# UltronAI/Depth-VO-Feat

Hardware: AMD Instinct MI355X
Metric: KITTI 256x832 stereo-seq samples/sec fwd+bwd (higher is better)
Workload: dtype f32

## Files before the change

__graft_entry__.py:

```python
import os
import subprocess
import sys

ROOT = os.path.dirname(os.path.abspath(__file__))
PKG = os.path.join(ROOT, "depth-vo-feat_amd")


def _paths():
    for p in (PKG, ROOT):
        if p not in sys.path:
            sys.path.insert(0, p)


def build():
    subprocess.run(["make", "-C", os.path.join(PKG, "csrc"), "-j4"], check=True)
    subprocess.run(["make", "-C", os.path.join(PKG, "csrc"), "TUNING=1", "-j4"], check=True)
    assert os.path.exists(os.path.join(PKG, "dvf", "libdvf_hip_tuning.so"))
    _paths()
    from dvf import lib as L
    lib = L.lib()
    assert lib.dvf_version() >= 100
    import DispNetS, PoseExpNet, PoseExpNet_sfm, inverse_warp, loss_functions, loss_functions_sfm
    import dvf.engine, dvf.steps


def smoke():
    _paths()
    import torch
    from oracle import nets as onets
    from oracle import steps as osteps
    import DispNetS
    import PoseExpNet
    from dvf.engine import FlatAdam
    from dvf.steps import unsupervise_losses
    from dvf.synthetic import synthetic_batch
    assert torch.cuda.is_available(), "smoke() needs the GPU: the product path has no CPU fallback"
    dev = torch.device("cuda:0")
    b, h, w = 1, 64, 128
    dsd = onets.fill_params(onets.dispnet_layers(), seed=1)
    psd = onets.fill_params(onets.posenet_layers(6, 6, 2, True), seed=2)
    disp, pose = DispNetS.DispNetS(), PoseExpNet.PoseExpNet(output_exp=True)
    disp.load_state_dict({k: v.clone() for k, v in dsd.items()})
    pose.load_state_dict({k: v.clone() for k, v in psd.items()})
    disp.to(dev).train()
    pose.to(dev).train()
    opt = FlatAdam(list(pose.parameters()) + list(disp.parameters()), lr=1e-3, weight_decay=1e-8)
    loss, terms = unsupervise_losses(disp, pose, synthetic_batch(b, h, w, seed=1234, device=dev))
    opt.zero_grad()
    loss.backward()
    opt.step()
    torch.cuda.synchronize()
    ref, _, _ = osteps.step_unsupervise(dsd, psd, osteps.synthetic_batch(b, h, w, seed=1234))
    for k in ("img", "smooth", "total"):
        err = abs(float(terms[k]) - float(ref[k])) / abs(float(ref[k]))
        assert err < 1e-4, (k, float(terms[k]), float(ref[k]))
    for name, net, sd in (("disp", disp, dsd), ("pose", pose, psd)):
        for k, v in net.state_dict().items():
            n0 = float(sd[k].double().norm())
            assert abs(float(v.double().norm().cpu()) - n0) <= 1e-4 * max(n0, 1e-12), (name, k)
    print("smoke ok: loss %.6f (oracle %.6f)" % (float(terms["total"]), float(ref["total"])))


if __name__ == "__main__":
    build()
    if "--smoke" in sys.argv:
        smoke()
```

depth-vo-feat_amd/csrc/conv_pipe.h:

```cpp
#pragma once
#include "dvf_common.h"
#include "conv_epilogue.h"

namespace dvfp {

#ifdef DVF_TUNING
#define DVF_STAMP(a, var) do { if ((a).stamps) asm volatile("s_memtime %0\n\ts_waitcnt lgkmcnt(0)" : "=s"(var) :: "memory"); } while (0)
#define DVF_STAMP_RT(a, var) do { if ((a).stamps) asm volatile("s_memrealtime %0\n\ts_waitcnt lgkmcnt(0)" : "=s"(var) :: "memory"); } while (0)
#define DVF_STAMPS_ON 1
#else
#define DVF_STAMP(a, var) do { } while (0)
#define DVF_STAMP_RT(a, var) do { } while (0)
#define DVF_STAMPS_ON 0
#endif

typedef __attribute__((address_space(3))) void lds_void_t;

__device__ __forceinline__ __amdgpu_buffer_rsrc_t tensor_rsrc(const void *p) {
    const uint64_t v = reinterpret_cast<uint64_t>(p);
    const unsigned lo = __builtin_amdgcn_readfirstlane((unsigned)v), hi = __builtin_amdgcn_readfirstlane((unsigned)(v >> 32));
    return __builtin_amdgcn_make_buffer_rsrc(reinterpret_cast<void *>(((uint64_t)hi << 32) | lo), 0, 0x7FFFFFF0, 0x00020000);
}
constexpr unsigned OOB = 0x80000000u;
__device__ __forceinline__ float bload(__amdgpu_buffer_rsrc_t r, unsigned voff, unsigned soff) {
    return __builtin_bit_cast(float, __builtin_amdgcn_raw_buffer_load_b32(r, voff, soff, 0));
}

struct PClass { int py, px, by, bx, TA, TB, OHc, OWc, SL, NTG; unsigned wp_off; };

struct PipeArgs {
    const float *in[DVF_MAX_SEGS];
    int segC[DVF_MAX_SEGS];
    int nseg;
    const float *wp;
    const float *bias;
    float *out;
    int M, N, IH, IW, OH, OW;
    int OS, IS, ncls;
    PClass cls[4];
    int act;
    float alpha, beta;
    int KS, NCH, out_mode, NG;
    int64_t ws_slice;
    int lsw, lsh, TGX, TGY, BW, BH, BN, tilesX, tilesY;
    int x4;
    int blk;
    int SLmax, PSRmax, NST;
    int dbg;
    unsigned long long *stamps;
    const float *mask;
};

__host__ __device__ inline int pipe_row_stride(int RSu, int SW, int SH, int IS) {
    if (SH == 1 || SW >= 32 || (SW % IS) != 0) return RSu;
    const int mod = 32 / IS, want = (SW / IS) % mod;
    const int padded = RSu + ((want - RSu % mod) + mod) % mod;
    return (padded * 8 <= RSu * 9) ? padded : RSu;
}

struct PipeGeo { int PH, PW, PWH, RS, PSR, NPI, XA; };
__host__ __device__ inline PipeGeo pipe_geo(int BH, int BW, int BN, int IS, int TA, int TB, int SW, int SH, int x4 = 0, int bx = 0) {
    PipeGeo g;
    g.PH = (BH - 1) * IS + TA;
    g.PW = (BW - 1) * IS + TB;
    g.PWH = (g.PW + 1) >> 1;
    g.XA = 0;
    if (x4) {
        g.XA = ((bx % 4) + 4) % 4;
        int rs = (g.XA + g.PW + 3) & ~3;
        if (SH > 1 && SW < 32 && (SW & 3) == 0) {
            int padded = rs;
            while (((padded * IS) & 31) != ((SW * IS) & 31) && padded < rs + 32) padded += 4;
            if (((padded * IS) & 31) == ((SW * IS) & 31) && padded * 8 <= rs * 9) rs = padded;
        }
        g.RS = rs;
        g.PSR = (BN * g.PH * g.RS + 255) & ~255;
        g.NPI = g.PSR >> 8;
        return g;
    }
    g.RS = pipe_row_stride(IS == 2 ? 2 * g.PWH : g.PW, SW, SH, IS);
    g.PSR = (BN * g.PH * g.RS + 63) & ~63;
    g.NPI = g.PSR >> 6;
    return g;
}

template <int V> struct fvec;
template <> struct fvec<1> { typedef float type; };
template <> struct fvec<2> { typedef float type __attribute__((ext_vector_type(2))); };
template <> struct fvec<4> { typedef float type __attribute__((ext_vector_type(4))); };

constexpr int PIPE_THREADS = 384;
constexpr int PIPE_THREADS_4P = 512;
constexpr int PIPE_MAXNPI = 32;

template <int MT, int NT, int WM, int CKH, int TBU, int BLK = 0, int NPMAX = PIPE_MAXNPI>
__global__ __launch_bounds__(PIPE_THREADS_4P) __attribute__((amdgpu_waves_per_eu(NPMAX < PIPE_MAXNPI ? 4 : 0)))
void conv_pipe_kernel(const PipeArgs a) {
    constexpr int CK = 2 * CKH, VW = CKH >= 4 ? 4 : CKH, CPG = CKH / VW, MTW = MT * WM;
    constexpr int UNITF = TBU * MTW * 64 * VW;
    static_assert(NPMAX >= 6 && NPMAX <= PIPE_MAXNPI, "by_np dispatches exact piece counts up to 6");
    typedef typename fvec<VW>::type avec;
    extern __shared__ __attribute__((aligned(16))) float smem[];
    const int stage_floats = a.SLmax + CK * a.PSRmax;
    const int tid = threadIdx.x, lane = tid & 63, nl = lane & 31, kh = lane >> 5;
    const int wave = __builtin_amdgcn_readfirstlane(tid >> 6);
    const int zper = gridDim.z / a.ncls;
    const int zc = blockIdx.z / zper, zr = blockIdx.z - zc * zper;
    const int ng = zr / a.KS, ks = zr - ng * a.KS;
    const PClass c = a.cls[zc];
    const int tX = blockIdx.x % a.tilesX, tY = blockIdx.x / a.tilesX;
    const int oy0 = tY * a.BH, ox0 = tX * a.BW, n0 = ng * a.BN;
    if (oy0 >= c.OHc || ox0 >= c.OWc) return;
    const int mb = blockIdx.y;
    const int SW = 1 << a.lsw, SH = 1 << a.lsh;
    const PipeGeo geo = pipe_geo(a.BH, a.BW, a.BN, a.IS, c.TA, TBU, SW, SH, a.x4, c.bx);
    const int RS = geo.RS, PSR = geo.PSR, PWH = geo.PWH;
    const int g_begin = (int)(((int64_t)a.NCH * ks) / a.KS), g_end = (int)(((int64_t)a.NCH * (ks + 1)) / a.KS);
    unsigned long long t_entry = 0, r_entry = 0;
    const int lin_block = (blockIdx.z * gridDim.y + blockIdx.y) * gridDim.x + blockIdx.x;
    DVF_STAMP(a, t_entry);
    DVF_STAMP_RT(a, r_entry);

    if (wave >= 4) {
        auto U = [](int v) __attribute__((always_inline)) { return __builtin_amdgcn_readfirstlane(v); };
        __builtin_amdgcn_s_setprio(3);
        const int nprod = U((int)(blockDim.x >> 6) - 4), pidx = wave - 4;
        const int par = U(nprod == 2 ? pidx : (pidx >> 1));
        const int half = U(nprod == 2 ? 0 : (pidx & 1)), nhalf = U(nprod == 2 ? 1 : 2);
        const int NWP = U(c.SL >> 8);
        const int iy0 = U(oy0 * a.IS + c.by), ix0 = U(ox0 * a.IS + c.bx);
        const int sfl = U(stage_floats), PSRu = U(PSR), NPIu = U(geo.NPI), SLu = U(c.SL), SLmaxu = U(a.SLmax);
        const unsigned wbase = (unsigned)U((int)(c.wp_off + (unsigned)(mb * a.NCH) * (unsigned)c.SL));
        const __amdgpu_buffer_rsrc_t rs_w = tensor_rsrc(a.wp);
        auto issue_w = [&](int g, int st) __attribute__((always_inline)) {
            if (DVF_DBG(a, 2)) return;
            float *wl = smem + st * sfl;
            unsigned so = ((wbase + (unsigned)g * (unsigned)SLu) << 2) + ((unsigned)half << 10);
            float *dst = wl + (half << 8);
            for (int p = half; p < NWP; p += nhalf) {
                __builtin_amdgcn_raw_ptr_buffer_load_lds(rs_w, (lds_void_t *)dst, 16, (unsigned)lane << 4, so, 0, 0);
                so += (unsigned)nhalf << 10;
                dst += nhalf << 8;
            }
        };
        const int D = U(a.NST - 1), nchunks = U(g_end - g_begin), g0 = U(g_begin);
        auto stage_of = [&](int x) __attribute__((always_inline)) { return D == 1 ? (x & 1) : x % 3; };
        if DVF_DBG(a, 8) return;
        for (int x = 0; x < D; ++x)
            if (x < nchunks && (x & 1) == par) issue_w(g0 + x, stage_of(x));

        unsigned pvf[NPMAX];
        unsigned pbn4[(NPMAX + 3) / 4];
#pragma unroll
        for (int q = 0; q < (NPMAX + 3) / 4; ++q) pbn4[q] = 0u;
        {
            const int per_img = geo.PH * RS;
            const float inv_img = 1.0f / (float)per_img, inv_rs = 1.0f / (float)RS;
#pragma unroll
            for (int kk = 0; kk < NPMAX; ++kk) {
                pvf[kk] = OOB;
                if (kk < NPIu) {
                    const int p = a.x4 ? (((kk << 6) + lane) << 2) : ((kk << 6) + lane);
                    int bn = (int)((float)p * inv_img);
                    bn += (p - bn * per_img >= per_img) - (p - bn * per_img < 0);
                    const int rem = p - bn * per_img;
                    int row = (int)((float)rem * inv_rs);
                    row += (rem - row * RS >= RS) - (rem - row * RS < 0);
                    const int col = rem - row * RS;
                    int cs = col - geo.XA;
                    bool ok = (bn < a.BN) && (n0 + bn < a.N);
                    if (a.IS == 2 && !a.x4) {
                        cs = col < PWH ? 2 * col : 2 * (col - PWH) + 1;
                        ok = ok && (col < 2 * PWH);
                    }
                    if (!a.x4) ok = ok && (cs < geo.PW);
                    const int iy = iy0 + row, ix = ix0 + cs;
                    ok = ok && (iy >= 0) && (iy < a.IH) && (ix >= 0) && (ix < a.IW);
                    pvf[kk] = ok ? (unsigned)((iy * a.IW + ix) << 2) : OOB;
                    pbn4[kk >> 2] |= (ok ? (unsigned)bn : 0u) << ((kk & 3) * 8);
                }
            }
        }
        const __amdgpu_buffer_rsrc_t rs_zero = __builtin_amdgcn_make_buffer_rsrc(
            const_cast<float *>(a.wp), 0, 0, 0x00020000);
        const unsigned plane = (unsigned)U((a.IH * a.IW) << 2);
        int iseg = -1, iseg_first = 0, iseg_end = 0, segc = 0;
        __amdgpu_buffer_rsrc_t rs_in = rs_zero;
        unsigned img_cur = 0u;
        auto enter_segment = [&](int g) __attribute__((always_inline)) {
            while (g >= iseg_end) {
                ++iseg;
                iseg_first = iseg_end;
                iseg_end += (a.segC[iseg] + CK - 1) / CK;
            }
            iseg = U(iseg); iseg_first = U(iseg_first); iseg_end = U(iseg_end);
            segc = U(a.segC[iseg]);
            rs_in = tensor_rsrc(a.in[iseg]);
            const unsigned img = (unsigned)segc * plane;
            if (a.BN > 1) {
                const unsigned delta = img - img_cur;
#pragma unroll
                for (int kk = 0; kk < NPMAX; ++kk)
                    if (kk < NPIu) pvf[kk] = (pvf[kk] >> 31) ? OOB : pvf[kk] + ((pbn4[kk >> 2] >> ((kk & 3) * 8)) & 255u) * delta;
            }
            img_cur = img;
        };
        auto issue_p = [&](int g, int st, auto lanec, auto npc, auto exactc) __attribute__((always_inline)) {
            constexpr int LB = decltype(lanec)::value, NP = decltype(npc)::value;
            constexpr bool EXACT = decltype(exactc)::value;
            constexpr int PSH = LB == 16 ? 8 : 6;
            if (g >= iseg_end) enter_segment(g);
            const int c0 = U((g - iseg_first) * CK);
            const int nch = U(min(CK, segc - c0));
            float *dst = smem + st * sfl + SLmaxu + half * PSRu;
            unsigned soff = (unsigned)U((int)((unsigned)(n0 * segc + c0 + half) * plane));
            auto dma = [&](__amdgpu_buffer_rsrc_t r, float *d, unsigned vo, unsigned so) __attribute__((always_inline)) {
                if constexpr (LB == 16) __builtin_amdgcn_raw_ptr_buffer_load_lds(r, (lds_void_t *)d, 16, vo, so, 0, 0);
                else __builtin_amdgcn_raw_ptr_buffer_load_lds(r, (lds_void_t *)d, 4, vo, so, 0, 0);
            };
            int ci = half;
            if (DVF_DBG(a, 32)) {
                for (; ci < nch; ci += nhalf) {
#pragma unroll
                    for (int kk = 0; kk < NP; ++kk)
                        if (EXACT || kk < NPIu) dma(rs_in, dst + (kk << PSH), (unsigned)lane * LB, (unsigned)(kk << (PSH + 2)));
                    dst += nhalf * PSRu;
                }
            }
            for (; ci < nch; ci += nhalf) {
#pragma unroll
                for (int kk = 0; kk < NP; ++kk)
                    if (EXACT || kk < NPIu) dma(rs_in, dst + (kk << PSH), pvf[kk], soff);
                dst += nhalf * PSRu;
                soff += (unsigned)nhalf * plane;
            }
            for (; ci < CK; ci += nhalf) {
#pragma unroll
                for (int kk = 0; kk < NP; ++kk)
                    if (EXACT || kk < NPIu) dma(rs_zero, dst + (kk << PSH), pvf[kk], 0u);
                dst += nhalf * PSRu;
            }
        };
        using std::integral_constant;
        unsigned long long p0 = 0, p1 = 0, p2 = 0, p3 = 0, w_vm = 0, w_bar = 0, w_iss = 0;
        auto chunk_loop = [&](auto lanec, auto npc, auto exactc) __attribute__((always_inline)) {
            if (!DVF_DBG(a, 1))
                for (int x = 0; x < D; ++x)
                    if (x < nchunks && (x & 1) == par) issue_p(g0 + x, stage_of(x), lanec, npc, exactc);
            for (int x = 0; x < nchunks; ++x) {
                DVF_STAMP(a, p0);
                if ((x & 1) == par) asm volatile("s_waitcnt vmcnt(0)" ::: "memory");
                DVF_STAMP(a, p1);
                __builtin_amdgcn_s_barrier();
                DVF_STAMP(a, p2);
                const int nx = x + D;
                if (nx < nchunks && (nx & 1) == par) {
                    issue_w(g0 + nx, stage_of(nx));
                    if (!DVF_DBG(a, 1)) issue_p(g0 + nx, stage_of(nx), lanec, npc, exactc);
                }
                DVF_STAMP(a, p3);
                w_vm += p1 - p0; w_bar += p2 - p1; w_iss += p3 - p2;
            }
        };
        auto by_np = [&](auto lanec) __attribute__((always_inline)) {
            switch (NPIu) {
                case 1: chunk_loop(lanec, integral_constant<int, 1>{}, std::true_type{}); break;
                case 2: chunk_loop(lanec, integral_constant<int, 2>{}, std::true_type{}); break;
                case 3: chunk_loop(lanec, integral_constant<int, 3>{}, std::true_type{}); break;
                case 4: chunk_loop(lanec, integral_constant<int, 4>{}, std::true_type{}); break;
                case 5: chunk_loop(lanec, integral_constant<int, 5>{}, std::true_type{}); break;
                case 6: chunk_loop(lanec, integral_constant<int, 6>{}, std::true_type{}); break;
                default:
                    if constexpr (NPMAX > 12) {
                        if (NPIu <= 12) chunk_loop(lanec, integral_constant<int, 12>{}, std::false_type{});
                        else chunk_loop(lanec, integral_constant<int, NPMAX>{}, std::false_type{});
                    } else {
                        chunk_loop(lanec, integral_constant<int, NPMAX>{}, std::false_type{});
                    }
            }
        };
        if (a.x4) by_np(integral_constant<int, 16>{});
        else by_np(integral_constant<int, 4>{});
        if (DVF_STAMPS_ON && a.stamps && pidx == 0 && lane == 0) {
            a.stamps[8 * lin_block + 5] = w_vm; a.stamps[8 * lin_block + 6] = w_bar; a.stamps[8 * lin_block + 7] = w_iss;
        }
        return;
    }

    const int wm = wave % WM, wn = wave / WM;
    float *bias_lds = smem + a.NST * stage_floats;
    if (tid < 32 * MTW) {
        const int mm = mb * (32 * MTW) + tid;
        bias_lds[tid] = (a.bias && a.out_mode == OUT_FUSED && mm < a.M) ? a.bias[mm] : 0.f;
    }
    const int NU = c.NTG * CPG;
    int opy[NT], opx[NT], opn[NT];
    constexpr bool LR = NPMAX < PIPE_MAXNPI;
    int bj[NT][LR ? 1 : VW];
    const int pxl = nl & (SW - 1), pyl = (nl >> a.lsw) & (SH - 1), pnl = nl >> (a.lsw + a.lsh);
    auto tile_pos = [&](int i, int pxv, int pyv, int pnv) __attribute__((always_inline)) {
        const int q = wn * NT + i, tx = q % a.TGX, tyn = q / a.TGX, ty = tyn % a.TGY, tn = tyn / a.TGY;
        const int SN = 32 >> (a.lsw + a.lsh);
        opy[i] = ty * SH + pyv;
        opx[i] = tx * SW + pxv;
        opn[i] = tn * SN + pnv;
    };
#pragma unroll
    for (int i = 0; i < NT; ++i) {
        tile_pos(i, pxl, pyl, pnl);
        const int bbase = kh * PSR + (opn[i] * geo.PH + opy[i] * a.IS) * RS + (a.x4 ? geo.XA + opx[i] * a.IS : opx[i]);
#pragma unroll
        for (int j = 0; j < (LR ? 1 : VW); ++j) bj[i][j] = bbase + j * 2 * PSR;
    }
    f32x16 acc[MT][NT];
    f32x16 asum[BLK ? MT : 1][BLK ? NT : 1];
#pragma unroll
    for (int m = 0; m < MT; ++m)
#pragma unroll
        for (int i = 0; i < NT; ++i)
#pragma unroll
            for (int r = 0; r < 16; ++r) {
                acc[m][i][r] = 0.f;
                if constexpr (BLK) asum[m][i][r] = 0.f;
            }

    auto consume = [&](int st, auto isc, auto tbec) {
        constexpr int IS = decltype(isc)::value, TBE = decltype(tbec)::value;
        const float *wl = smem + st * stage_floats;
        const float *patch = wl + a.SLmax;
        const float *ap = wl + (wm * MT) * 64 * VW + lane * VW;
        avec af[2][MT];
        float bf[2][TBE][NT][VW];
        int lta = 0, lcpg = 0, lk = 0;
        auto load_bj = [&](auto bufc, auto jc) {
            constexpr int buf = decltype(bufc)::value, j = decltype(jc)::value;
            const float *prow0 = patch + (lta * RS + (lcpg * (2 * VW) + (LR ? 2 * j : 0)) * PSR);
#pragma unroll
            for (int i = 0; i < NT; ++i) {
                const float *prow = prow0 + bj[i][LR ? 0 : j];
                if constexpr (IS == 1) {
#pragma unroll
                    for (int u = 0; u < TBE; ++u) bf[buf][u][i][j] = prow[u];
                } else {
                    const float *prow2 = prow + PWH;
#pragma unroll
                    for (int u = 0; u < TBE; ++u) bf[buf][u][i][j] = (u & 1) ? prow2[u >> 1] : prow[u >> 1];
                }
            }
        };
        auto load_b = [&](auto bufc) {
            load_bj(bufc, std::integral_constant<int, 0>{});
            if constexpr (VW > 1) load_bj(bufc, std::integral_constant<int, 1>{});
            if constexpr (VW > 2) load_bj(bufc, std::integral_constant<int, 2>{});
            if constexpr (VW > 3) load_bj(bufc, std::integral_constant<int, 3>{});
        };
        auto load_a = [&](auto tpc, int unit, auto uc) {
            constexpr int tp = decltype(tpc)::value, u = decltype(uc)::value;
            const float *aptr = ap + unit * UNITF;
#pragma unroll
            for (int m = 0; m < MT; ++m) af[tp][m] = *reinterpret_cast<const avec *>(aptr + (u * MTW + m) * 64 * VW);
        };
        auto advance = [&]() {
            ++lk;
            const bool wrap = (lcpg + 1 == CPG);
            lcpg = wrap ? 0 : lcpg + 1;
            lta += wrap ? 1 : 0;
        };
        auto mma_j = [&](auto bufc, auto tpc, auto uc, auto jc) {
            constexpr int buf = decltype(bufc)::value, tp = decltype(tpc)::value, u = decltype(uc)::value, j = decltype(jc)::value;
#pragma unroll
            for (int m = 0; m < MT; ++m) {
                float av;
                if constexpr (VW == 1) av = af[tp][m]; else av = af[tp][m][j];
#pragma unroll
                for (int i = 0; i < NT; ++i)
                    acc[m][i] = __builtin_amdgcn_mfma_f32_32x32x2f32(av, bf[buf][u][i][j], acc[m][i], 0, 0, 0);
            }
        };
        using B0 = std::integral_constant<int, 0>;
        using B1 = std::integral_constant<int, 1>;
        auto step = [&](auto bufc, auto nbufc, auto pbc, auto uc) {
            constexpr int u = decltype(uc)::value, tp = (decltype(pbc)::value + u) & 1;
            using TP = std::integral_constant<int, tp>;
            mma_j(bufc, TP{}, uc, std::integral_constant<int, 0>{});
            __builtin_amdgcn_sched_barrier(0);
            if constexpr (u + 1 < TBE) load_a(std::integral_constant<int, tp ^ 1>{}, lk - 1, std::integral_constant<int, u + 1>{});
            else load_a(std::integral_constant<int, tp ^ 1>{}, lk, std::integral_constant<int, 0>{});
            if constexpr (u == 0) load_bj(nbufc, std::integral_constant<int, 0>{});
            __builtin_amdgcn_sched_barrier(0);
            if constexpr (VW > 1) {
                mma_j(bufc, TP{}, uc, std::integral_constant<int, 1>{});
                __builtin_amdgcn_sched_barrier(0);
                if constexpr (u == 0) { load_bj(nbufc, std::integral_constant<int, 1>{}); __builtin_amdgcn_sched_barrier(0); }
            }
            if constexpr (VW > 2) {
                mma_j(bufc, TP{}, uc, std::integral_constant<int, 2>{});
                __builtin_amdgcn_sched_barrier(0);
                if constexpr (u == 0) { load_bj(nbufc, std::integral_constant<int, 2>{}); __builtin_amdgcn_sched_barrier(0); }
            }
            if constexpr (VW > 3) {
                mma_j(bufc, TP{}, uc, std::integral_constant<int, 3>{});
                __builtin_amdgcn_sched_barrier(0);
                if constexpr (u == 0) { load_bj(nbufc, std::integral_constant<int, 3>{}); __builtin_amdgcn_sched_barrier(0); }
            }
        };
        auto unit = [&](auto bufc, auto nbufc, auto pbc) {
            step(bufc, nbufc, pbc, std::integral_constant<int, 0>{});
            if constexpr (TBE > 1) step(bufc, nbufc, pbc, std::integral_constant<int, 1>{});
            if constexpr (TBE > 2) step(bufc, nbufc, pbc, std::integral_constant<int, 2>{});
            if constexpr (TBE > 3) step(bufc, nbufc, pbc, std::integral_constant<int, 3>{});
            if constexpr (TBE > 4) step(bufc, nbufc, pbc, std::integral_constant<int, 4>{});
            if constexpr (TBE > 5) step(bufc, nbufc, pbc, std::integral_constant<int, 5>{});
            if constexpr (TBE > 6) step(bufc, nbufc, pbc, std::integral_constant<int, 6>{});
            advance();
        };
        load_b(B0{});
        load_a(B0{}, 0, std::integral_constant<int, 0>{});
        advance();
        __builtin_amdgcn_sched_barrier(0);
        for (int k = 0; k < NU; k += 2) {
            unit(B0{}, B1{}, std::integral_constant<int, 0>{});
            if (k + 1 < NU) unit(B1{}, B0{}, std::integral_constant<int, TBE & 1>{});
        }
    };

    unsigned long long t_loop0 = 0, t_loop1 = 0, tb0 = 0, tb1 = 0, w_bar = 0;
    DVF_STAMP(a, t_loop0);
    if (!DVF_DBG(a, 8)) {
        using IS1 = std::integral_constant<int, 1>;
        using IS2 = std::integral_constant<int, 2>;
        using TBfull = std::integral_constant<int, TBU>;
        using TBless = std::integral_constant<int, (TBU > 1 ? TBU - 1 : 1)>;
        if constexpr (LR) {
            static_assert(!BLK, "the low-register form has no second accumulator set");
            auto chunks = [&](auto isc, auto tbec) __attribute__((always_inline)) {
                int st = 0;
                for (int g = g_begin; g < g_end; ++g) {
                    DVF_STAMP(a, tb0);
                    __syncthreads();
                    DVF_STAMP(a, tb1);
                    w_bar += tb1 - tb0;
                    if (!DVF_DBG(a, 4)) consume(st, isc, tbec);
                    st = (st + 1 == a.NST) ? 0 : st + 1;
                }
            };
            if (a.IS == 2 && !a.x4) chunks(IS2{}, TBfull{});
            else if (TBU > 1 && c.TB == TBU - 1 && !DVF_DBG(a, 64)) chunks(IS1{}, TBless{});
            else chunks(IS1{}, TBfull{});
        } else {
            int st = 0, since = 0;
            for (int g = g_begin; g < g_end; ++g) {
                DVF_STAMP(a, tb0);
                __syncthreads();
                DVF_STAMP(a, tb1);
                w_bar += tb1 - tb0;
                if (!DVF_DBG(a, 4)) {
                    if (a.IS == 2 && !a.x4) consume(st, IS2{}, TBfull{});
                    else if (TBU > 1 && c.TB == TBU - 1 && !DVF_DBG(a, 64)) consume(st, IS1{}, TBless{});
                    else consume(st, IS1{}, TBfull{});
                }
                if constexpr (BLK) {
                    if (++since == a.blk) {
                        since = 0;
#pragma unroll
                        for (int m = 0; m < MT; ++m)
#pragma unroll
                            for (int i = 0; i < NT; ++i) {
                                asum[m][i] += acc[m][i];
#pragma unroll
                                for (int r = 0; r < 16; ++r) acc[m][i][r] = 0.f;
                            }
                    }
                }
                st = (st + 1 == a.NST) ? 0 : st + 1;
            }
        }
    }
    if constexpr (BLK) {
#pragma unroll
        for (int m = 0; m < MT; ++m)
#pragma unroll
            for (int i = 0; i < NT; ++i) acc[m][i] += asum[m][i];
    }

    if constexpr (LR) {
        int nlv = nl;
        asm volatile("" : "+v"(nlv));
#pragma unroll
        for (int i = 0; i < NT; ++i) tile_pos(i, nlv & (SW - 1), (nlv >> a.lsw) & (SH - 1), nlv >> (a.lsw + a.lsh));
    }
    DVF_STAMP(a, t_loop1);
    auto stamp_out = [&]() {
        if (DVF_STAMPS_ON && a.stamps && wave == 0) {
            unsigned long long t_end = 0, r_end = 0;
            asm volatile("s_waitcnt vmcnt(0)" ::: "memory");
            DVF_STAMP(a, t_end);
            DVF_STAMP_RT(a, r_end);
            if (lane == 0) {
                unsigned long long *o = a.stamps + 8 * lin_block;
                o[0] = t_loop0 - t_entry; o[1] = t_loop1 - t_loop0; o[2] = w_bar; o[3] = t_end - t_loop1; o[4] = r_end - r_entry;
            }
        }
    };
    if DVF_DBG(a, 16) { stamp_out(); return; }
    const int m0 = mb * (32 * MTW) + wm * (32 * MT);
    const int64_t HW = (int64_t)a.OH * a.OW;
    if (a.mask && a.out_mode == OUT_FUSED) {
        float *outp = a.out;
#pragma unroll
        for (int i = 0; i < NT; ++i) {
            const int oy = oy0 + opy[i], ox = ox0 + opx[i], n = n0 + opn[i];
            const int Y = oy * a.OS + c.py, X = ox * a.OS + c.px;
            const bool pok = (oy < c.OHc) && (ox < c.OWc) && (Y < a.OH) && (X < a.OW) && (opn[i] < a.BN) && (n < a.N);
            const int64_t base = ((int64_t)n * a.M + m0 + 4 * kh) * HW + (int64_t)Y * a.OW + X;
            float mk[MT][16];
#pragma unroll
            for (int m = 0; m < MT; ++m)
#pragma unroll
                for (int r = 0; r < 16; ++r) {
                    const int ml = m * 32 + (r & 3) + 8 * (r >> 2);
                    const bool ok = pok && (m0 + 4 * kh + ml < a.M);
                    mk[m][r] = a.mask[ok ? base + (int64_t)ml * HW : 0];
                }
#pragma unroll
            for (int m = 0; m < MT; ++m) {
#pragma unroll
                for (int r = 0; r < 16; ++r) {
                    const int ml = m * 32 + (r & 3) + 8 * (r >> 2);
                    if (pok && m0 + 4 * kh + ml < a.M) {
                        outp[base + (int64_t)ml * HW] = mk[m][r] > 0.f ? acc[m][i][r] : 0.f;
                    }
                }
            }
        }
        stamp_out();
        return;
    }
    store_tile<MT, NT>(
        acc, a.out + (a.out_mode == OUT_WS ? (int64_t)ks * a.ws_slice : 0), nullptr, a.out_mode, a.act, a.alpha, a.beta, m0, kh, a.M, HW,
        [&](int i, int64_t &off) __attribute__((always_inline)) {
            const int oy = oy0 + opy[i], ox = ox0 + opx[i], n = n0 + opn[i];
            const int Y = oy * a.OS + c.py, X = ox * a.OS + c.px;
            off = ((int64_t)n * a.M + m0 + 4 * kh) * HW + (int64_t)Y * a.OW + X;
            return (oy < c.OHc) && (ox < c.OWc) && (Y < a.OH) && (X < a.OW) && (opn[i] < a.BN) && (n < a.N);
        },
        [&](int ml) __attribute__((always_inline)) { return bias_lds[wm * (32 * MT) + 4 * kh + ml]; });
    stamp_out();
}

template <int MT, int NT, int WM>
int launch_pipe_family(const PipeArgs &a, int CKH, int TBU, dim3 grid, size_t lds, hipStream_t st, int threads);
template <int MT, int NT, int WM>
int launch_pipe_family_lr(const PipeArgs &a, int CKH, int TBU, dim3 grid, size_t lds, hipStream_t st, int threads);

constexpr int PIPE_LR_NPI = 12;
constexpr size_t PIPE_LR_LDS = 80 * 1024;
constexpr bool pipe_has_lr(int MT, int NT, int WM, int CKH, int TBU) {
    if (WM != 1) return false;
    if (MT == 2) return NT == 1;
    return !(NT == 2 && CKH == 4 && TBU >= 5);
}

template <int MT, int NT, int WM, int CKH, int TBU>
constexpr bool pipe_has_blk() {
#ifdef DVF_TUNING
    return true;
#else
    return MT == 2 && NT == 1 && WM == 1 && CKH >= 4 && TBU >= 2 && TBU <= 4;
#endif
}

template <int MT, int NT, int WM, int CKH, int TBU, int BLK, int NPMAX = PIPE_MAXNPI>
inline int launch_pipe_blk(const PipeArgs &a, dim3 grid, size_t lds, hipStream_t st, int threads) {
    static bool big_lds = false;
    if (lds > 64 * 1024 && !big_lds) {
        if (hipFuncSetAttribute(reinterpret_cast<const void *>(&conv_pipe_kernel<MT, NT, WM, CKH, TBU, BLK, NPMAX>),
                                hipFuncAttributeMaxDynamicSharedMemorySize, 160 * 1024) != hipSuccess)
            return DVF_ERR_LAUNCH;
        big_lds = true;
    }
    conv_pipe_kernel<MT, NT, WM, CKH, TBU, BLK, NPMAX><<<grid, threads, lds, st>>>(a);
    return hipGetLastError() == hipSuccess ? DVF_OK : DVF_ERR_LAUNCH;
}

template <int MT, int NT, int WM, int CKH, int TBU, bool LR>
inline int launch_pipe_one(const PipeArgs &a, dim3 grid, size_t lds, hipStream_t st, int threads) {
    if constexpr (LR) {
        if constexpr (pipe_has_lr(MT, NT, WM, CKH, TBU)) {
            if (a.blk || lds > PIPE_LR_LDS) return DVF_ERR_UNSUPPORTED;
            return launch_pipe_blk<MT, NT, WM, CKH, TBU, 0, PIPE_LR_NPI>(a, grid, lds, st, threads);
        } else {
            return DVF_ERR_UNSUPPORTED;
        }
    } else {
        if (a.blk) {
            if constexpr (pipe_has_blk<MT, NT, WM, CKH, TBU>()) return launch_pipe_blk<MT, NT, WM, CKH, TBU, 1>(a, grid, lds, st, threads);
            else return DVF_ERR_UNSUPPORTED;
        }
        return launch_pipe_blk<MT, NT, WM, CKH, TBU, 0>(a, grid, lds, st, threads);
    }
}

template <int MT, int NT, int WM, int CKH, bool LR>
inline int launch_pipe_tbu(const PipeArgs &a, int TBU, dim3 grid, size_t lds, hipStream_t st, int threads) {
    switch (TBU) {
        case 1: return launch_pipe_one<MT, NT, WM, CKH, 1, LR>(a, grid, lds, st, threads);
        case 2: return launch_pipe_one<MT, NT, WM, CKH, 2, LR>(a, grid, lds, st, threads);
        case 3: return launch_pipe_one<MT, NT, WM, CKH, 3, LR>(a, grid, lds, st, threads);
        case 4: return launch_pipe_one<MT, NT, WM, CKH, 4, LR>(a, grid, lds, st, threads);
        case 5: if constexpr (CKH <= 4 && WM == 1) return launch_pipe_one<MT, NT, WM, CKH, 5, LR>(a, grid, lds, st, threads); else return DVF_ERR_UNSUPPORTED;
        case 7: if constexpr (CKH <= 4 && WM == 1) return launch_pipe_one<MT, NT, WM, CKH, 7, LR>(a, grid, lds, st, threads); else return DVF_ERR_UNSUPPORTED;
        default: return DVF_ERR_UNSUPPORTED;
    }
}

#define DVF_PIPE_FAMILY_(NAME, LR, MT, NT, WM)                                                                   \
    template <>                                                                                                  \
    int NAME<MT, NT, WM>(const PipeArgs &a, int CKH, int TBU, dim3 grid, size_t lds, hipStream_t st, int threads) { \
        switch (CKH) {                                                                                           \
            case 2: return launch_pipe_tbu<MT, NT, WM, 2, LR>(a, TBU, grid, lds, st, threads);                   \
            case 4: return launch_pipe_tbu<MT, NT, WM, 4, LR>(a, TBU, grid, lds, st, threads);                   \
            case 8: return launch_pipe_tbu<MT, NT, WM, 8, LR>(a, TBU, grid, lds, st, threads);                   \
            default: return DVF_ERR_UNSUPPORTED;                                                                 \
        }                                                                                                        \
    }
#define DVF_PIPE_FAMILY(MT, NT, WM) DVF_PIPE_FAMILY_(launch_pipe_family, false, MT, NT, WM)
#define DVF_PIPE_FAMILY_LR(MT, NT, WM) DVF_PIPE_FAMILY_(launch_pipe_family_lr, true, MT, NT, WM)

}
```

depth-vo-feat_amd/csrc/conv_pipe_host.h:

```cpp
#pragma once
#include <string.h>
#include "dvf_common.h"
#include "conv_pipe.h"
#include "conv_op.h"

namespace {

using dvfp::PClass;
using dvfp::PipeArgs;
using dvfp::PipeGeo;
using dvfp::pipe_geo;
using dvfp::PIPE_MAXNPI;
using dvfp::OUT_FUSED;
using dvfp::OUT_ATOMIC;
using dvfp::OUT_WS;

struct alignas(8) PackArgsBody {
    const float *w;
    float *wp;
    int w_mode;
    int Mtot, Rtot, KK, m_base, M;
    int nseg, segC[DVF_MAX_SEGS];
    int ncls, NCH, CK, MB, VW, TBU;
    int TB[4], TA[4];
// ... 351 lines not shown
    static const int big_lds_kb = dvf_tune("DVF_PIPE_BIGLDS_KB") ? atoi(dvf_tune("DVF_PIPE_BIGLDS_KB")) : 150;
    const size_t PIPE_LDS_BUDGET = (nblk * KS0 <= 256 ? big_lds_kb : 76) * 1024;
    struct Depth { int ok, CK, NST, PSRmax; size_t lds; int NPImax; };
    auto depth_for = [&](int x4) {
        Depth d{0, 0, 3, 0, 0, 0};
        for (int i = 0; i < ncls; ++i) {
            const PipeGeo g = pipe_geo(a.BH, a.BW, a.BN, a.IS, cls[i].TA, TBU, SW, SH, x4, cls[i].bx);
            if (g.NPI > PIPE_MAXNPI) return d;
            d.PSRmax = g.PSR > d.PSRmax ? g.PSR : d.PSRmax;
            d.NPImax = g.NPI > d.NPImax ? g.NPI : d.NPImax;
        }
        auto lds_bytes = [&](int CK) { return ((size_t)d.NST * (slab(CK, TAmax) + (size_t)CK * d.PSRmax) + MB) * 4; };
        int CK = TBU >= 5 ? 8 : 16;
        while (CK > 4 && lds_bytes(CK) > PIPE_LDS_BUDGET) CK >>= 1;
        while (CK > 4 && CK / 2 >= maxc) CK >>= 1;
        if (lds_bytes(CK) > PIPE_LDS_BUDGET) {
            d.NST = 2;
            if (lds_bytes(CK) > PIPE_LDS_BUDGET && PIPE_LDS_BUDGET < 150 * 1024) {
                d.NST = 3;
                if (lds_bytes(CK) > 150 * 1024) d.NST = 2;
                if (lds_bytes(CK) > 150 * 1024) return d;
            }
        }
        if (ov.on && ov.CK) { CK = ov.CK; d.NST = 3; if (lds_bytes(CK) > 150 * 1024) d.NST = 2; }
        if (ov.on && ov.NST) d.NST = ov.NST;
        if ((CK != 4 && CK != 8 && CK != 16) || lds_bytes(CK) > 150 * 1024) return d;
        d.ok = 1; d.CK = CK; d.lds = lds_bytes(CK);
        return d;
    };
    int want_x4 = (a.IW % 4 == 0 && (a.BW * a.IS) % 4 == 0) ? 1 : 0;
    if (const char *e = dvf_tune("DVF_PIPE_X4")) want_x4 = want_x4 && atoi(e) != 0;
    const Depth d1 = depth_for(0), d4 = want_x4 ? depth_for(1) : Depth{0, 0, 3, 0, 0, 0};
    static const bool x4_force = dvf_tune("DVF_PIPE_X4") && atoi(dvf_tune("DVF_PIPE_X4")) == 2;
    const bool use4 = d4.ok && (!d1.ok || x4_force || (d4.CK >= d1.CK && d4.NST >= d1.NST));
    const Depth dd = use4 ? d4 : d1;
    if (!dd.ok) return DVF_ERR_UNSUPPORTED;
    a.x4 = use4 ? 1 : 0;
    a.PSRmax = dd.PSRmax;
    const int CK = dd.CK, NST = dd.NST;
    a.NST = NST;
    a.SLmax = slab(CK, TAmax);
    a.NCH = 0;
    for (int s = 0; s < a.nseg; ++s) a.NCH += cdiv(a.segC[s], CK);
    const int mblocks = cdiv(a.M, MB);
    unsigned off = 0;
    for (int i = 0; i < ncls; ++i) {
        const ClassSpec &c = cls[i];
        const int SL = slab(CK, c.TA);
        a.cls[i] = PClass{c.py, c.px, c.by, c.bx, c.TA, c.TB, c.OHc, c.OWc, SL, c.TA, off};
        const int64_t nf = (int64_t)mblocks * a.NCH * SL;
        if ((int64_t)off + nf >= ((int64_t)1 << 29)) return DVF_ERR_UNSUPPORTED;
        off += (unsigned)nf;
    }
    pl.packed_floats = off;
    int KS = KS0;
    if (ov.on && ov.KS) KS = ov.KS;
    if (KS > a.NCH) KS = a.NCH;
    if (KS < 1) KS = 1;
    if ((int64_t)a.NG * KS * ncls > 65535) return DVF_ERR_UNSUPPORTED;
    a.KS = KS;
    pl.ws_floats = (op.covers && KS > 1) ? (int64_t)KS * a.N * a.M * a.OH * a.OW : 0;
    pl.reduce_kpar = KS >= 8 && (int64_t)a.OH * a.OW < ((int64_t)1 << 30);
    for (int s2 = 0; s2 < a.nseg; ++s2)
        if ((int64_t)a.N * a.segC[s2] * a.IH * a.IW * 4 >= ((int64_t)1 << 31) - 16) return DVF_ERR_UNSUPPORTED;
    pl.MT = MT; pl.NT = NT; pl.WM = WM; pl.CKH = CK / 2; pl.TBU = TBU; pl.lds = dd.lds;
    pl.pack_lds = (size_t)32 * ((CK * op.KK) | 1) * sizeof(float);
    if (pl.pack_lds > 64 * 1024) return DVF_ERR_UNSUPPORTED;
    pl.grid = dim3(a.tilesX * a.tilesY, mblocks, a.NG * KS * ncls);
    {
        const int per_chunk = CK * TAmax * TBmax;
        const int64_t kseq = (int64_t)cdiv(a.NCH, KS) * per_chunk;
        static const int blk_knob = dvf_tune("DVF_PIPE_BLK") ? atoi(dvf_tune("DVF_PIPE_BLK")) : -1;
        static const int blk_terms = dvf_tune("DVF_PIPE_BLKT") ? atoi(dvf_tune("DVF_PIPE_BLKT")) : 0;
        const bool deep = MT == 2 && NT == 1 && WM == 1 && CK >= 8 && TBU >= 2 && TBU <= 4 && kseq >= 512 &&
                          ((int64_t)pl.grid.x * pl.grid.y * pl.grid.z <= 256 || pl.lds > 76 * 1024);
        int every = blk_terms > 0 ? (blk_terms + per_chunk / 2) / per_chunk : 1;
        if (every < 1) every = 1;
        a.blk = blk_knob == 0 ? 0 : blk_knob > 0 ? blk_knob : blk_terms > 0 ? (kseq >= 384 ? every : 0) : (deep ? 1 : 0);
    }
    {
        const int64_t nblocks_total = (int64_t)pl.grid.x * pl.grid.y * pl.grid.z;
        static const bool no4p = dvf_tune("DVF_PIPE_NO4P") != nullptr;
        static const int mt1_4p = dvf_tune("DVF_PIPE_MT1_4P") ? atoi(dvf_tune("DVF_PIPE_MT1_4P")) : 1;
        pl.threads = (!no4p && (pl.lds > 76 * 1024 || nblocks_total <= 256 || (MT == 1 && mt1_4p))) ? dvfp::PIPE_THREADS_4P : dvfp::PIPE_THREADS;
        pl.npi = dd.NPImax;
        const bool lr_fits = !a.blk && dd.NPImax <= dvfp::PIPE_LR_NPI && pl.lds <= dvfp::PIPE_LR_LDS &&
                             dvfp::pipe_has_lr(MT, NT, WM, CK / 2, TBU);
        pl.lr = lr_fits && nblocks_total > 256;
        if (const char *e = dvf_tune("DVF_PIPE_LR")) pl.lr = lr_fits && atoi(e) != 0;
    }
    return DVF_OK;
}

int launch_pipe(const PipeArgs &a, const PipePlan &pl, hipStream_t st) {
    using dvfp::launch_pipe_family;
    if (pl.lr) {
        if (pl.WM != 1) return DVF_ERR_UNSUPPORTED;
        if (pl.MT == 2) return dvfp::launch_pipe_family_lr<2, 1, 1>(a, pl.CKH, pl.TBU, pl.grid, pl.lds, st, pl.threads);
        return pl.NT == 2 ? dvfp::launch_pipe_family_lr<1, 2, 1>(a, pl.CKH, pl.TBU, pl.grid, pl.lds, st, pl.threads)
                          : dvfp::launch_pipe_family_lr<1, 1, 1>(a, pl.CKH, pl.TBU, pl.grid, pl.lds, st, pl.threads);
    }
    if (pl.WM == 2) {
        if (pl.NT != 1) return DVF_ERR_UNSUPPORTED;
        return pl.MT == 2 ? launch_pipe_family<2, 1, 2>(a, pl.CKH, pl.TBU, pl.grid, pl.lds, st, pl.threads)
                          : launch_pipe_family<1, 1, 2>(a, pl.CKH, pl.TBU, pl.grid, pl.lds, st, pl.threads);
    }
    if (pl.WM != 1) return DVF_ERR_UNSUPPORTED;
    if (pl.MT == 2 && pl.NT == 2) return DVF_ERR_UNSUPPORTED;
    if (pl.MT == 2) return launch_pipe_family<2, 1, 1>(a, pl.CKH, pl.TBU, pl.grid, pl.lds, st, pl.threads);
    if (pl.NT == 2) return launch_pipe_family<1, 2, 1>(a, pl.CKH, pl.TBU, pl.grid, pl.lds, st, pl.threads);
    return launch_pipe_family<1, 1, 1>(a, pl.CKH, pl.TBU, pl.grid, pl.lds, st, pl.threads);
}

int run_pipe(const ConvOp &op, const PipePlan &pl, const ConvIO &io, const float *packed, float *ws, int64_t ws_floats,
             hipStream_t st) {
    PipeArgs a = pl.a;
    for (int s = 0; s < a.nseg; ++s) {
        a.in[s] = io.in[s];
        if (a.x4 && (reinterpret_cast<uintptr_t>(a.in[s]) & 15)) return DVF_ERR_UNSUPPORTED;
    }
    a.wp = packed; a.bias = io.bias; a.mask = io.mask;
    const int mode = out_mode_of(op.covers, a.KS, ws, ws_floats, pl.ws_floats);
    int rc = prepare_output(a, mode, io.out, ws, st);
    if (rc) return rc;
    if (const char *e = dvf_tune("DVF_DBG")) a.dbg = atoi(e);
    a.stamps = nullptr;
#ifdef DVF_TUNING
    if (dvf_tune("DVF_STAMPS")) {
        const size_t nb = (size_t)pl.grid.x * pl.grid.y * pl.grid.z;
        if (!g_stamp_buf && hipMalloc(&g_stamp_buf, STAMP_MAX_BLOCKS * 64) != hipSuccess) return DVF_ERR_LAUNCH;
        if (nb <= STAMP_MAX_BLOCKS) {
            if (hipMemsetAsync(g_stamp_buf, 0, nb * 64, st) != hipSuccess) return DVF_ERR_LAUNCH;
            a.stamps = g_stamp_buf;
            g_stamp_blocks = (int)nb;
        }
    }
#endif
    dvf_plan_note(DVF_K_PIPE, pl.MT, pl.NT, pl.WM, 2 * pl.CKH, pl.TBU, a.KS, a.BN, a.NST, pl.threads, (int)pl.lds, mode | (a.ncls << 4) | (a.x4 << 8) | ((a.blk ? 1 : 0) << 9) | (pl.lr << 10) | (pl.npi << 11));
    if (dvf_tune("DVF_PIPE_DEBUG"))
        fprintf(stderr, "[pipe] M %d chunks %d N %d out %dx%d cls %d | MT %d NT %d WM %d CK %d TBU %d KS %d BN %d tile %dx%d "
                "(sub %dx%d) grid %ux%ux%u lds %zu x%d mode %d\n", a.M, a.NCH, a.N, a.OH, a.OW, a.ncls, pl.MT, pl.NT, pl.WM,
                2 * pl.CKH, pl.TBU, a.KS, a.BN, a.BH, a.BW, 1 << a.lsh, 1 << a.lsw, pl.grid.x, pl.grid.y, pl.grid.z, pl.lds, a.NST, mode);
    rc = launch_pipe(a, pl, st);
    return rc ? rc : finish_output(a, pl.reduce_kpar, ws, io.out, st);
}

PackArgs pack_job(const ConvOp &op, const PipePlan &pl, const float *w, float *packed, int *blocks) {
    const PipeArgs &a = pl.a;
    PackArgs p{};
    p.w = w; p.wp = packed; p.w_mode = op.w_mode; p.Mtot = op.Mtot; p.Rtot = op.Rtot; p.KK = op.KK;
    p.m_base = op.m_base; p.M = a.M; p.nseg = a.nseg;
    for (int s = 0; s < a.nseg; ++s) p.segC[s] = a.segC[s];
    p.ncls = op.ncls; p.NCH = a.NCH; p.CK = 2 * pl.CKH; p.MB = 32 * pl.MT * pl.WM; p.VW = pl.CKH >= 4 ? 4 : pl.CKH;
    p.TBU = pl.TBU;
    for (int c = 0; c < op.ncls; ++c) {
        p.SL[c] = a.cls[c].SL;
        p.TB[c] = op.cls[c].TB;
        p.TA[c] = op.cls[c].TA;
        p.wp_off[c] = a.cls[c].wp_off;
        for (int t = 0; t < op.cls[c].TA * op.cls[c].TB; ++t) p.tapmap[c][t] = (signed char)op.cls[c].tapmap[t];
    }
    *blocks = a.NCH * cdiv(a.M, p.MB) * (p.MB >> 5);
    return p;
}

int launch_pack(const ConvOp &op, const PipePlan &pl, const float *w, float *packed, hipStream_t st) {
    int blocks;
    const PackArgs p = pack_job(op, pl, w, packed, &blocks);
    conv_pack_kernel<<<dim3(p.NCH, blocks / p.NCH), 256, pl.pack_lds, st>>>(p);
    DVF_LAUNCH_CHECK();
    return DVF_OK;
}

}
```

depth-vo-feat_amd/csrc/conv_pipe_inst_a.hip:

```cpp
#include "conv_pipe.h"
namespace dvfp {
DVF_PIPE_FAMILY(1, 1, 1)
DVF_PIPE_FAMILY(1, 2, 1)
}
```

depth-vo-feat_amd/csrc/conv_pipe_inst_c.hip:

```cpp
#include "conv_pipe.h"
namespace dvfp {
DVF_PIPE_FAMILY(1, 1, 2)
DVF_PIPE_FAMILY(2, 1, 2)
}
```

Measured before the change: 664.0.

## Group two K-chunks per barrier in pipelined conv for small grids

Adds a grouping mode (G=2) to the non-low-register pipelined convolution kernel. Producers load two chunks per barrier into four LDS stage slots, and consumers process both chunks in one consume call. This halves the number of block-wide barriers on long-K, low-occupancy launches (at most 256 blocks, at least 16 chunks per split). In exchange it uses more LDS and changes the pipelining depth. It also splits the template instantiations into separate files so they build in parallel, and runs the two make builds concurrently.

```diff
diff --git a/__graft_entry__.py b/__graft_entry__.py
--- a/__graft_entry__.py
+++ b/__graft_entry__.py
@@ -13,8 +13,9 @@
 
 
 def build():
-    subprocess.run(["make", "-C", os.path.join(PKG, "csrc"), "-j4"], check=True)
-    subprocess.run(["make", "-C", os.path.join(PKG, "csrc"), "TUNING=1", "-j4"], check=True)
+    makes = [subprocess.Popen(["make", "-C", os.path.join(PKG, "csrc"), "-j4"] + extra) for extra in ([], ["TUNING=1"])]
+    for m in [m for m in makes if m.wait() != 0]:
+        raise subprocess.CalledProcessError(m.returncode, m.args)
     assert os.path.exists(os.path.join(PKG, "dvf", "libdvf_hip_tuning.so"))
     _paths()
     from dvf import lib as L
diff --git a/depth-vo-feat_amd/csrc/conv_pipe.h b/depth-vo-feat_amd/csrc/conv_pipe.h
--- a/depth-vo-feat_amd/csrc/conv_pipe.h
+++ b/depth-vo-feat_amd/csrc/conv_pipe.h
@@ -46,6 +46,7 @@
     int x4;
     int blk;
     int SLmax, PSRmax, NST;
+    int G;
     int dbg;
     unsigned long long *stamps;
     const float *mask;
@@ -116,6 +117,10 @@
     const PipeGeo geo = pipe_geo(a.BH, a.BW, a.BN, a.IS, c.TA, TBU, SW, SH, a.x4, c.bx);
     const int RS = geo.RS, PSR = geo.PSR, PWH = geo.PWH;
     const int g_begin = (int)(((int64_t)a.NCH * ks) / a.KS), g_end = (int)(((int64_t)a.NCH * (ks + 1)) / a.KS);
+    constexpr bool LR = NPMAX < PIPE_MAXNPI;
+    const int GG = LR ? 1 : __builtin_amdgcn_readfirstlane(a.G > 1 ? 2 : 1);
+    const int nslot = LR ? a.NST : __builtin_amdgcn_readfirstlane(GG > 1 ? 4 : a.NST);
+    const int nbar = LR ? g_end - g_begin : __builtin_amdgcn_readfirstlane((g_end - g_begin + GG - 1) / GG);
     unsigned long long t_entry = 0, r_entry = 0;
     const int lin_block = (blockIdx.z * gridDim.y + blockIdx.y) * gridDim.x + blockIdx.x;
     DVF_STAMP(a, t_entry);
@@ -143,11 +148,18 @@
                 dst += nhalf << 8;
             }
         };
-        const int D = U(a.NST - 1), nchunks = U(g_end - g_begin), g0 = U(g_begin);
-        auto stage_of = [&](int x) __attribute__((always_inline)) { return D == 1 ? (x & 1) : x % 3; };
+        const int D = U(GG > 1 ? 1 : a.NST - 1), nchunks = U(g_end - g_begin), g0 = U(g_begin);
+        auto stage_of = [&](int x) __attribute__((always_inline)) {
+            if constexpr (LR) return D == 1 ? (x & 1) : x % 3;
+            else return GG > 1 ? (x & 3) : D == 1 ? (x & 1) : x % 3;
+        };
+        auto for_group = [&](int q, auto f) __attribute__((always_inline)) {
+            if constexpr (LR) f(q);
+            else for (int x = q * GG; x < min(q * GG + GG, nchunks); ++x) f(x);
+        };
         if DVF_DBG(a, 8) return;
-        for (int x = 0; x < D; ++x)
-            if (x < nchunks && (x & 1) == par) issue_w(g0 + x, stage_of(x));
+        for (int q = 0; q < D; ++q)
+            if (q < nbar && (q & 1) == par) for_group(q, [&](int x) __attribute__((always_inline)) { issue_w(g0 + x, stage_of(x)); });
 
         unsigned pvf[NPMAX];
         unsigned pbn4[(NPMAX + 3) / 4];
@@ -245,18 +257,21 @@
         unsigned long long p0 = 0, p1 = 0, p2 = 0, p3 = 0, w_vm = 0, w_bar = 0, w_iss = 0;
         auto chunk_loop = [&](auto lanec, auto npc, auto exactc) __attribute__((always_inline)) {
             if (!DVF_DBG(a, 1))
-                for (int x = 0; x < D; ++x)
-                    if (x < nchunks && (x & 1) == par) issue_p(g0 + x, stage_of(x), lanec, npc, exactc);
-            for (int x = 0; x < nchunks; ++x) {
+                for (int q = 0; q < D; ++q)
+                    if (q < nbar && (q & 1) == par)
+                        for_group(q, [&](int x) __attribute__((always_inline)) { issue_p(g0 + x, stage_of(x), lanec, npc, exactc); });
+            for (int q = 0; q < nbar; ++q) {
                 DVF_STAMP(a, p0);
-                if ((x & 1) == par) asm volatile("s_waitcnt vmcnt(0)" ::: "memory");
+                if ((q & 1) == par) asm volatile("s_waitcnt vmcnt(0)" ::: "memory");
                 DVF_STAMP(a, p1);
                 __builtin_amdgcn_s_barrier();
                 DVF_STAMP(a, p2);
-                const int nx = x + D;
-                if (nx < nchunks && (nx & 1) == par) {
-                    issue_w(g0 + nx, stage_of(nx));
-                    if (!DVF_DBG(a, 1)) issue_p(g0 + nx, stage_of(nx), lanec, npc, exactc);
+                const int nq = q + D;
+                if (nq < nbar && (nq & 1) == par) {
+                    for_group(nq, [&](int x) __attribute__((always_inline)) {
+                        issue_w(g0 + x, stage_of(x));
+                        if (!DVF_DBG(a, 1)) issue_p(g0 + x, stage_of(x), lanec, npc, exactc);
+                    });
                 }
                 DVF_STAMP(a, p3);
                 w_vm += p1 - p0; w_bar += p2 - p1; w_iss += p3 - p2;
@@ -288,14 +303,13 @@
     }
 
     const int wm = wave % WM, wn = wave / WM;
-    float *bias_lds = smem + a.NST * stage_floats;
+    float *bias_lds = smem + nslot * stage_floats;
     if (tid < 32 * MTW) {
         const int mm = mb * (32 * MTW) + tid;
         bias_lds[tid] = (a.bias && a.out_mode == OUT_FUSED && mm < a.M) ? a.bias[mm] : 0.f;
     }
     const int NU = c.NTG * CPG;
     int opy[NT], opx[NT], opn[NT];
-    constexpr bool LR = NPMAX < PIPE_MAXNPI;
     int bj[NT][LR ? 1 : VW];
     const int pxl = nl & (SW - 1), pyl = (nl >> a.lsw) & (SH - 1), pnl = nl >> (a.lsw + a.lsh);
     auto tile_pos = [&](int i, int pxv, int pyv, int pnv) __attribute__((always_inline)) {
@@ -324,8 +338,12 @@
                 if constexpr (BLK) asum[m][i][r] = 0.f;
             }
 
-    auto consume = [&](int st, auto isc, auto tbec) {
+    [[maybe_unused]] int since = 0;
+    auto consume = [&](int st, int nck, auto isc, auto tbec) {
         constexpr int IS = decltype(isc)::value, TBE = decltype(tbec)::value;
+        const int NUT = LR ? NU : nck * NU;
+        const int ajump = stage_floats - NU * UNITF;
+        int poff = 0;
         const float *wl = smem + st * stage_floats;
         const float *patch = wl + a.SLmax;
         const float *ap = wl + (wm * MT) * 64 * VW + lane * VW;
@@ -334,7 +352,7 @@
         int lta = 0, lcpg = 0, lk = 0;
         auto load_bj = [&](auto bufc, auto jc) {
             constexpr int buf = decltype(bufc)::value, j = decltype(jc)::value;
-            const float *prow0 = patch + (lta * RS + (lcpg * (2 * VW) + (LR ? 2 * j : 0)) * PSR);
+            const float *prow0 = patch + (LR ? 0 : poff) + (lta * RS + (lcpg * (2 * VW) + (LR ? 2 * j : 0)) * PSR);
 #pragma unroll
             for (int i = 0; i < NT; ++i) {
                 const float *prow = prow0 + bj[i][LR ? 0 : j];
@@ -356,7 +374,7 @@
         };
         auto load_a = [&](auto tpc, int unit, auto uc) {
             constexpr int tp = decltype(tpc)::value, u = decltype(uc)::value;
-            const float *aptr = ap + unit * UNITF;
+            const float *aptr = ap + unit * UNITF + ((!LR && unit >= NU) ? ajump : 0);
 #pragma unroll
             for (int m = 0; m < MT; ++m) af[tp][m] = *reinterpret_cast<const avec *>(aptr + (u * MTW + m) * 64 * VW);
         };
@@ -365,6 +383,24 @@
             const bool wrap = (lcpg + 1 == CPG);
             lcpg = wrap ? 0 : lcpg + 1;
             lta += wrap ? 1 : 0;
+            if constexpr (!LR) {
+                if (lk == NU && nck > 1) { lta = 0; poff = stage_floats; }
+            }
+        };
+        auto chunk_end = [&](int done) {
+            if constexpr (BLK) {
+                if ((done == NU || done == NUT) && ++since == a.blk) {
+                    since = 0;
+#pragma unroll
+                    for (int m = 0; m < MT; ++m)
+#pragma unroll
+                        for (int i = 0; i < NT; ++i) {
+                            asum[m][i] += acc[m][i];
+#pragma unroll
+                            for (int r = 0; r < 16; ++r) acc[m][i][r] = 0.f;
+                        }
+                }
+            }
         };
         auto mma_j = [&](auto bufc, auto tpc, auto uc, auto jc) {
             constexpr int buf = decltype(bufc)::value, tp = decltype(tpc)::value, u = decltype(uc)::value, j = decltype(jc)::value;
@@ -418,9 +454,13 @@
         load_a(B0{}, 0, std::integral_constant<int, 0>{});
         advance();
         __builtin_amdgcn_sched_barrier(0);
-        for (int k = 0; k < NU; k += 2) {
+        for (int k = 0; k < NUT; k += 2) {
             unit(B0{}, B1{}, std::integral_constant<int, 0>{});
-            if (k + 1 < NU) unit(B1{}, B0{}, std::integral_constant<int, TBE & 1>{});
+            chunk_end(k + 1);
+            if (k + 1 < NUT) {
+                unit(B1{}, B0{}, std::integral_constant<int, TBE & 1>{});
+                chunk_end(k + 2);
+            }
         }
     };
 
@@ -431,50 +471,25 @@
         using IS2 = std::integral_constant<int, 2>;
         using TBfull = std::integral_constant<int, TBU>;
         using TBless = std::integral_constant<int, (TBU > 1 ? TBU - 1 : 1)>;
-        if constexpr (LR) {
-            static_assert(!BLK, "the low-register form has no second accumulator set");
-            auto chunks = [&](auto isc, auto tbec) __attribute__((always_inline)) {
-                int st = 0;
-                for (int g = g_begin; g < g_end; ++g) {
-                    DVF_STAMP(a, tb0);
-                    __syncthreads();
-                    DVF_STAMP(a, tb1);
-                    w_bar += tb1 - tb0;
-                    if (!DVF_DBG(a, 4)) consume(st, isc, tbec);
-                    st = (st + 1 == a.NST) ? 0 : st + 1;
-                }
-            };
-            if (a.IS == 2 && !a.x4) chunks(IS2{}, TBfull{});
-            else if (TBU > 1 && c.TB == TBU - 1 && !DVF_DBG(a, 64)) chunks(IS1{}, TBless{});
-            else chunks(IS1{}, TBfull{});
-        } else {
-            int st = 0, since = 0;
-            for (int g = g_begin; g < g_end; ++g) {
+        static_assert(!(LR && BLK), "the low-register form has no second accumulator set");
+        auto chunks = [&](auto isc, auto tbec) __attribute__((always_inline)) {
+            int st = 0, x = 0;
+            const int nchunks = g_end - g_begin;
+            for (int q = 0; q < nbar; ++q) {
                 DVF_STAMP(a, tb0);
                 __syncthreads();
                 DVF_STAMP(a, tb1);
                 w_bar += tb1 - tb0;
-                if (!DVF_DBG(a, 4)) {
-                    if (a.IS == 2 && !a.x4) consume(st, IS2{}, TBfull{});
-                    else if (TBU > 1 && c.TB == TBU - 1 && !DVF_DBG(a, 64)) consume(st, IS1{}, TBless{});
-                    else consume(st, IS1{}, TBfull{});
-                }
-                if constexpr (BLK) {
-                    if (++since == a.blk) {
-                        since = 0;
-#pragma unroll
-                        for (int m = 0; m < MT; ++m)
-#pragma unroll
-                            for (int i = 0; i < NT; ++i) {
-                                asum[m][i] += acc[m][i];
-#pragma unroll
-                                for (int r = 0; r < 16; ++r) acc[m][i][r] = 0.f;
-                            }
-                    }
-                }
-                st = (st + 1 == a.NST) ? 0 : st + 1;
-            }
-        }
+                const int nck = LR ? 1 : min(GG, nchunks - x);
+                if (!DVF_DBG(a, 4)) consume(st, nck, isc, tbec);
+                x += nck;
+                st += nck;
+                if (st >= nslot) st -= nslot;
+            }
+        };
+        if (a.IS == 2 && !a.x4) chunks(IS2{}, TBfull{});
+        else if (TBU > 1 && c.TB == TBU - 1 && !DVF_DBG(a, 64)) chunks(IS1{}, TBless{});
+        else chunks(IS1{}, TBfull{});
     }
     if constexpr (BLK) {
 #pragma unroll
@@ -555,6 +570,7 @@
 
 constexpr int PIPE_LR_NPI = 12;
 constexpr size_t PIPE_LR_LDS = 80 * 1024;
+constexpr int PIPE_GROUP_MIN_CHUNKS = 16;
 constexpr bool pipe_has_lr(int MT, int NT, int WM, int CKH, int TBU) {
     if (WM != 1) return false;
     if (MT == 2) return NT == 1;
@@ -587,7 +603,7 @@
 inline int launch_pipe_one(const PipeArgs &a, dim3 grid, size_t lds, hipStream_t st, int threads) {
     if constexpr (LR) {
         if constexpr (pipe_has_lr(MT, NT, WM, CKH, TBU)) {
-            if (a.blk || lds > PIPE_LR_LDS) return DVF_ERR_UNSUPPORTED;
+            if (a.blk || a.G > 1 || lds > PIPE_LR_LDS) return DVF_ERR_UNSUPPORTED;
             return launch_pipe_blk<MT, NT, WM, CKH, TBU, 0, PIPE_LR_NPI>(a, grid, lds, st, threads);
         } else {
             return DVF_ERR_UNSUPPORTED;
diff --git a/depth-vo-feat_amd/csrc/conv_pipe_host.h b/depth-vo-feat_amd/csrc/conv_pipe_host.h
--- a/depth-vo-feat_amd/csrc/conv_pipe_host.h
+++ b/depth-vo-feat_amd/csrc/conv_pipe_host.h
@@ -457,12 +457,17 @@
         const int64_t nblocks_total = (int64_t)pl.grid.x * pl.grid.y * pl.grid.z;
         static const bool no4p = dvf_tune("DVF_PIPE_NO4P") != nullptr;
         static const int mt1_4p = dvf_tune("DVF_PIPE_MT1_4P") ? atoi(dvf_tune("DVF_PIPE_MT1_4P")) : 1;
-        pl.threads = (!no4p && (pl.lds > 76 * 1024 || nblocks_total <= 256 || (MT == 1 && mt1_4p))) ? dvfp::PIPE_THREADS_4P : dvfp::PIPE_THREADS;
         pl.npi = dd.NPImax;
         const bool lr_fits = !a.blk && dd.NPImax <= dvfp::PIPE_LR_NPI && pl.lds <= dvfp::PIPE_LR_LDS &&
                              dvfp::pipe_has_lr(MT, NT, WM, CK / 2, TBU);
         pl.lr = lr_fits && nblocks_total > 256;
         if (const char *e = dvf_tune("DVF_PIPE_LR")) pl.lr = lr_fits && atoi(e) != 0;
+        const size_t lds_g2 = (4 * ((size_t)a.SLmax + (size_t)CK * a.PSRmax) + MB) * 4;
+        const bool g_fits = NST == 3 && !pl.lr && lds_g2 <= (size_t)big_lds_kb * 1024 && lds_g2 <= 150 * 1024;
+        a.G = (g_fits && nblocks_total <= 256 && a.NCH / KS >= dvfp::PIPE_GROUP_MIN_CHUNKS) ? 2 : 1;
+        if (const char *e = dvf_tune("DVF_PIPE_GROUP")) a.G = (g_fits && atoi(e) >= 2) ? 2 : 1;
+        if (a.G == 2) pl.lds = lds_g2;
+        pl.threads = (!no4p && (pl.lds > 76 * 1024 || nblocks_total <= 256 || (MT == 1 && mt1_4p))) ? dvfp::PIPE_THREADS_4P : dvfp::PIPE_THREADS;
     }
     return DVF_OK;
 }
@@ -511,7 +516,7 @@
         }
     }
 #endif
-    dvf_plan_note(DVF_K_PIPE, pl.MT, pl.NT, pl.WM, 2 * pl.CKH, pl.TBU, a.KS, a.BN, a.NST, pl.threads, (int)pl.lds, mode | (a.ncls << 4) | (a.x4 << 8) | ((a.blk ? 1 : 0) << 9) | (pl.lr << 10) | (pl.npi << 11));
+    dvf_plan_note(DVF_K_PIPE, pl.MT, pl.NT, pl.WM, 2 * pl.CKH | ((a.G - 1) << 8), pl.TBU, a.KS, a.BN, a.NST, pl.threads, (int)pl.lds, mode | (a.ncls << 4) | (a.x4 << 8) | ((a.blk ? 1 : 0) << 9) | (pl.lr << 10) | (pl.npi << 11));
     if (dvf_tune("DVF_PIPE_DEBUG"))
         fprintf(stderr, "[pipe] M %d chunks %d N %d out %dx%d cls %d | MT %d NT %d WM %d CK %d TBU %d KS %d BN %d tile %dx%d "
                 "(sub %dx%d) grid %ux%ux%u lds %zu x%d mode %d\n", a.M, a.NCH, a.N, a.OH, a.OW, a.ncls, pl.MT, pl.NT, pl.WM,
diff --git a/depth-vo-feat_amd/csrc/conv_pipe_inst_a.hip b/depth-vo-feat_amd/csrc/conv_pipe_inst_a.hip
--- a/depth-vo-feat_amd/csrc/conv_pipe_inst_a.hip
+++ b/depth-vo-feat_amd/csrc/conv_pipe_inst_a.hip
@@ -1,5 +1,4 @@
 #include "conv_pipe.h"
 namespace dvfp {
 DVF_PIPE_FAMILY(1, 1, 1)
-DVF_PIPE_FAMILY(1, 2, 1)
 }
diff --git a/depth-vo-feat_amd/csrc/conv_pipe_inst_c.hip b/depth-vo-feat_amd/csrc/conv_pipe_inst_c.hip
--- a/depth-vo-feat_amd/csrc/conv_pipe_inst_c.hip
+++ b/depth-vo-feat_amd/csrc/conv_pipe_inst_c.hip
@@ -1,5 +1,4 @@
 #include "conv_pipe.h"
 namespace dvfp {
 DVF_PIPE_FAMILY(1, 1, 2)
-DVF_PIPE_FAMILY(2, 1, 2)
 }
diff --git a/depth-vo-feat_amd/csrc/conv_pipe_inst_f.hip b/depth-vo-feat_amd/csrc/conv_pipe_inst_f.hip
--- /dev/null
+++ b/depth-vo-feat_amd/csrc/conv_pipe_inst_f.hip
@@ -0,0 +1,4 @@
+#include "conv_pipe.h"
+namespace dvfp {
+DVF_PIPE_FAMILY(1, 2, 1)
+}
diff --git a/depth-vo-feat_amd/csrc/conv_pipe_inst_g.hip b/depth-vo-feat_amd/csrc/conv_pipe_inst_g.hip
--- /dev/null
+++ b/depth-vo-feat_amd/csrc/conv_pipe_inst_g.hip
@@ -0,0 +1,4 @@
+#include "conv_pipe.h"
+namespace dvfp {
+DVF_PIPE_FAMILY(2, 1, 2)
+}
```

Measured after the change: 665.4 (median of 2 runs). Within noise of the previous version (+0.2%).
